# AgoraIO-Community/Solo

Hardware: AMD Instinct MI355X
Metric: 40 ms frames/sec (encode+decode) per GPU; concurrent real-time WB streams @1/2/4/8 MI355X (higher is better)
Workload: dtype int32 fixed point (int16 PCM, Q-format arithmetic, bit-exact); 1 GPU; BASELINE configs[2]: 4096 synthetic 16 kHz WB streams, full encode -> two-description bitstream -...; streams_per_gpu=4096, input_workers=16, launch=single process

## Files before the change

solo_amd/csrc/solo_api.hip:

```cpp
#include <hip/hip_runtime.h>
#include <vector>
#include <stdio.h>
#include <stdlib.h>
#include <string.h>
#include <new>

#include "../../include/solo_mi355x.h"
#include "solo_dec.h"

#define SOLO_CHECK(expr)                                        \
    do {                                                        \
        hipError_t e_ = (expr);                                 \
        if (e_ != hipSuccess) return -(int32_t)e_;              \
    } while (0)

#include "solo_dec_kernels.h"
#include "solo_l0_probe.h"
#include "solo_send.h"
#include "solo_mix.h"
#include "solo_mix_shared.h"
#include "solo_mix_selected.h"
#include "solo_fanout.h"
#include "solo_recv_report.h"
#include "solo_migrate.h"
// ... 102 lines not shown
        for (int t = 0; t < trips; t++) {
            if (t) x = sx_add(sx_add(x, a), sx_add(f, sx_add(g, (i32)(u32)h)));
            SOLO_WAVEOPS_CHAIN(x)
        }
        ROW(9, a); ROW(10, b); ROW(11, c); ROW(12, d); ROW(13, e); ROW(14, f); ROW(15, g); ROW(16, (u32)h); ROW(17, (u32)((u64)h >> 32));
    }
#undef ROW
#endif
}

__global__ void __launch_bounds__(256) solo_stream_list_check_kernel(const i32* map, int n, int n_streams, u32* verdict, i32* status) {
    __shared__ int bad;
    if (threadIdx.x == 0) bad = 0;
    __syncthreads();
    int mine = 0;
    for (int i = threadIdx.x; i < n; i += 256) {
        const i32 v = map[i];
        if (v < 0 || v >= n_streams || (i > 0 && map[i - 1] >= v)) mine = 1;
    }
    if (mine) atomicOr(&bad, 1);
    __syncthreads();
    const int verdict_bad = bad;
    if (threadIdx.x == 0) *verdict = (u32)verdict_bad;
    if (verdict_bad && status)
        for (int i = threadIdx.x; i < n; i += 256) status[i] = -1;
}

extern "C" const solo_dec_ops* solo_nb_dec_ops() { return &solo_dec_ops_table; }
extern "C" const solo_dec_ops* solo_wb_dec_ops();

#ifdef SOLO_WITH_ENCODER
#include "solo_enc_ops.h"
extern "C" int solo_launch_gate(const unsigned int* flag, unsigned int target, void* hip_stream);
extern "C" const solo_enc_ops* solo_nb_enc_ops();
extern "C" const solo_enc_ops* solo_wb_enc_ops();
#endif

#define SOLO_MAX_CHUNKS 64
enum {
    SOLO_VERDICT_ENC = 0,
    SOLO_VERDICT_DEC = 2,
    SOLO_VERDICT_RING,
    SOLO_VERDICT_SEND,
    SOLO_VERDICT_MIX,
    SOLO_VERDICT_REPORT,
    SOLO_VERDICT_EXPORT,
    SOLO_VERDICT_IMPORT,
    SOLO_N_VERDICTS = SOLO_VERDICT_IMPORT + 2
};
struct solo_batch {
    int32_t n_streams;
    int32_t slot;
    int have_enc, have_dec;
    USER_Ctrl_enc enc_ctrl;
    USER_Ctrl_dec dec_ctrl;
    void* d_enc_state;
#ifdef SOLO_WITH_ENCODER
    const solo_enc_ops* eops;
#endif
    void* d_nsq_ring;
    hipEvent_t evDecDone;
    int dec_done_recorded;
    void* d_parsed;
    size_t parsed_bytes;
    int dec_pipe_ready, dec_split, dec_chunk, dec_first;
    size_t dec_scratch_cap;
    void* d_rc_scratch;
    size_t rc_scratch_bytes;
    void* d_enc_work;
    int32_t enc_work_packets;
    int timing;
    hipEvent_t evDec[2];
    int ev_ready, ev_enc, ev_dec;
    int pipe_ready, chunk_packets;
    hipStream_t sA, sB, sC;
    hipEvent_t evFork, evJoinA[2], evJoinC[2], evA[SOLO_MAX_CHUNKS], evB[SOLO_MAX_CHUNKS], evC[SOLO_MAX_CHUNKS];
    int async_join;
    unsigned int enc_seq;
    unsigned long long join_cap[2];
    int evC_valid;
    int last_np, last_cp;
    hipEvent_t tev[3][SOLO_MAX_CHUNKS][2];
    int tev_ready, last_chunks;
    unsigned int* d_started;
    unsigned int started_target[SOLO_MAX_CHUNKS];
    int group_streams;
    int gate;
    int persist;
    int persist_group;
    unsigned int* d_flags;
    unsigned int ticket;
    unsigned int final_wait_ticks;
    int front_defer;
    void* d_nsq_stage;
    void* d_front_scratch;
    const solo_dec_ops* dops;
    void* d_dec_state;
    uint8_t* d_recv_ring;
    uint32_t* d_recv_lens;
    int32_t* d_recv_play;
    uint32_t* d_recv_stats;
    int32_t recv_depth, recv_slot;
    uint32_t* d_recv_trk;
    int recv_track;
    int32_t* d_recv_sel;
    uint32_t* d_verdict;
    void* d_send_scratch;
// ... 990 lines not shown
        const int32_t r = solo_wait_in_flight(b, st);
        if (r) return r;
    }
    uint32_t* verdict = b->d_verdict + SOLO_VERDICT_IMPORT;
    SOLO_CHECK(launch_list_check(d_streams, n, b->n_streams, verdict, NULL, st));
    SOLO_CHECK(solo_migrate_import_launch(migrate_handle(b), d_streams, n, which, d_blob, (long long)blob_stride, (SxMigCount*)d_count, verdict, st));
    return 0;
}

#ifdef SOLO_WITH_ENCODER
static int32_t solo_enc_pipe_setup(solo_batch* b) {
    const solo_enc_ops* ops = b->eops;
    int lo = 0, hi = 0;
    (void)hipDeviceGetStreamPriorityRange(&lo, &hi);
    SOLO_CHECK(hipStreamCreateWithPriority(&b->sA, hipStreamNonBlocking, lo));
    SOLO_CHECK(hipStreamCreateWithPriority(&b->sB, hipStreamNonBlocking, hi));
    SOLO_CHECK(hipStreamCreateWithPriority(&b->sC, hipStreamNonBlocking, lo));
    SOLO_CHECK(hipEventCreateWithFlags(&b->evFork, hipEventDisableTiming));
    for (int i = 0; i < 2; i++) {
        SOLO_CHECK(hipEventCreateWithFlags(&b->evJoinA[i], hipEventDisableTiming));
        SOLO_CHECK(hipEventCreateWithFlags(&b->evJoinC[i], hipEventDisableTiming));
    }
    for (int c = 0; c < SOLO_MAX_CHUNKS; c++) {
        SOLO_CHECK(hipEventCreateWithFlags(&b->evA[c], hipEventDisableTiming));
        SOLO_CHECK(hipEventCreateWithFlags(&b->evB[c], hipEventDisableTiming));
        SOLO_CHECK(hipEventCreateWithFlags(&b->evC[c], hipEventDisableTiming));
    }
    int dev = 0, ncu = 0;
    SOLO_CHECK(hipGetDevice(&dev));
    SOLO_CHECK(hipDeviceGetAttribute(&ncu, hipDeviceAttributeMultiprocessorCount, dev));
    b->persist = env_int("SOLO_ENC_PERSIST", 0) != 0;
    b->chunk_packets = env_int("SOLO_ENC_CHUNK", 1);
    if (b->chunk_packets < 0) b->chunk_packets = 1;
    b->gate = getenv("SOLO_ENC_GATE") ? (env_int("SOLO_ENC_GATE", 0) != 0) : -1;
    const int g_env = env_int("SOLO_ENC_GROUP", -1);
    b->group_streams = g_env >= 0 ? g_env : 8192;
    b->persist_group = g_env > 0 ? ((g_env + 3) & ~3) : ((ops->front_per_cu * (ncu > 0 ? ncu : 256)) & ~3);
    if (b->persist_group < 4) b->persist_group = 4;
    {
        const long us = env_int("SOLO_ENC_FINAL_WAIT_US", 20000);
        b->front_defer = us < 0;
        b->final_wait_ticks = (unsigned int)((us < 0 ? 0 : (us > 10000000 ? 10000000 : us)) * 100);
    }
    {
        int gs = (b->group_streams > 0 && b->group_streams < b->n_streams) ? b->group_streams : b->n_streams;
        if (b->persist && b->persist_group > gs) gs = b->persist_group < b->n_streams ? b->persist_group : b->n_streams;
        SOLO_CHECK(hipMalloc(&b->d_nsq_ring, ops->nsq_ring_bytes(gs)));
    }
    SOLO_CHECK(hipMalloc((void**)&b->d_started, SOLO_MAX_CHUNKS * sizeof(unsigned int)));
    SOLO_CHECK(hipMemset(b->d_started, 0, SOLO_MAX_CHUNKS * sizeof(unsigned int)));
    memset(b->started_target, 0, sizeof(b->started_target));
    if (b->persist) {
        const size_t nflags = (size_t)b->n_streams * 2 + (size_t)b->n_streams / 4 + 1 + 4;
        SOLO_CHECK(hipMalloc((void**)&b->d_flags, nflags * sizeof(unsigned int)));
        SOLO_CHECK(hipMemset(b->d_flags, 0, nflags * sizeof(unsigned int)));
        const int gs = b->persist_group < b->n_streams ? b->persist_group : b->n_streams;
        SOLO_CHECK(hipMalloc(&b->d_front_scratch, ops->front_scratch_bytes(gs)));
        SOLO_CHECK(hipMalloc(&b->d_nsq_stage, ops->nsq_stage_bytes(gs)));
    }
    b->ticket = 0;
    b->pipe_ready = 1;
    return 0;
}

static int32_t solo_encode_persist(solo_batch* b, const int16_t* d_pcm, int32_t n_packets, uint8_t* d_bits, int16_t* d_nbytes, int32_t* d_status,
                                   hipStream_t st, void* nin, void* nout, void* cin) {
// ... 66 lines not shown
    SOLO_CHECK(lerr);
    SOLO_CHECK(hipGetLastError());
    return 0;
}

static int32_t solo_encode_impl(solo_batch_t* b, const int32_t* map, int32_t n, const int16_t* d_pcm, int32_t n_packets, uint8_t* d_bits, int16_t* d_nbytes,
                                int32_t* d_status, hipStream_t st) {
    const size_t np = (size_t)b->n_streams * (size_t)n_packets;
    const solo_enc_ops* ops = b->eops;
    if (map && (unsigned long long)b->n_streams * (unsigned long long)ops->state_bytes >= (1ull << 32)) return -1;
    const unsigned long long per_wave = 64ull / (unsigned long long)ops->nsq_workgroups(64);
    if (((per_wave - 1ull) * 2ull * (unsigned long long)n_packets + 1ull) * (unsigned long long)ops->nsq_out_bytes >= (1ull << 32)) return -1;
    const size_t sz_in = np * 2 * ops->nsq_in_bytes, sz_out = np * 2 * ops->nsq_out_bytes, sz_code = np * ops->code_in_bytes;
    if (n_packets > b->enc_work_packets) {
        SOLO_CHECK(hipStreamSynchronize(st));
        if (b->pipe_ready) { (void)hipStreamSynchronize(b->sA); (void)hipStreamSynchronize(b->sB); (void)hipStreamSynchronize(b->sC); }
        dev_free(b->d_enc_work);
        SOLO_CHECK(hipMalloc(&b->d_enc_work, sz_in + sz_out + sz_code + 256));
        b->enc_work_packets = n_packets;
    }
    void* nin = b->d_enc_work;
    void* nout = (char*)b->d_enc_work + ((sz_in + 63) & ~(size_t)63);
    void* cin = (char*)nout + ((sz_out + 63) & ~(size_t)63);
    void* states = b->d_enc_state;
    if (!b->pipe_ready) {
        const int32_t r = solo_enc_pipe_setup(b);
        if (r) return r;
    }
    if (!map && b->persist && n_packets >= 2) return solo_encode_persist(b, d_pcm, n_packets, d_bits, d_nbytes, d_status, st, nin, nout, cin);

    int cp = b->chunk_packets > 0 ? b->chunk_packets : n_packets;
    int nchunks = (n_packets + cp - 1) / cp;
    if (nchunks > SOLO_MAX_CHUNKS) { cp = (n_packets + SOLO_MAX_CHUNKS - 1) / SOLO_MAX_CHUNKS; nchunks = (n_packets + cp - 1) / cp; }
    {
        const int gs = (b->group_streams > 0 && b->group_streams < b->n_streams) ? b->group_streams : b->n_streams;
        SOLO_CHECK(grow_scratch(b->d_rc_scratch, b->rc_scratch_bytes, ops->rc_scratch_bytes(gs, cp), b->sC));
    }
    const bool tm_req = b->timing && b->tev_ready;
    const unsigned long long cap = stream_capture(st);
    if (b->enc_seq > 0 && b->join_cap[(b->enc_seq - 1u) & 1u] != cap) b->evC_valid = -1;
    uint32_t* verdict = NULL;
    if (map) {
        if (b->evC_valid > 0) b->evC_valid = 0;
        verdict = b->d_verdict + SOLO_VERDICT_ENC + (b->enc_seq & 1u);
        if (b->enc_seq >= 2 && b->join_cap[b->enc_seq & 1u] == cap) {
            SOLO_CHECK(hipStreamWaitEvent(st, b->evJoinA[b->enc_seq & 1u], 0));
            SOLO_CHECK(hipStreamWaitEvent(st, b->evJoinC[b->enc_seq & 1u], 0));
        }
        SOLO_CHECK(launch_list_check(map, n, b->n_streams, verdict, d_status, st));
    }
    if (b->evC_valid < 0) b->evC_valid = 0;
    else if (b->enc_seq > 0 && (b->last_np != n_packets || b->last_cp != cp || b->evC_valid == 0)) {
        SOLO_CHECK(hipStreamWaitEvent(b->sA, b->evJoinC[(b->enc_seq - 1u) & 1u], 0));
        SOLO_CHECK(hipStreamWaitEvent(b->sB, b->evJoinA[(b->enc_seq - 1u) & 1u], 0));
        b->evC_valid = 0;
    }
    b->last_np = n_packets;
    b->last_cp = cp;
    SOLO_CHECK(hipEventRecord(b->evFork, st));
    SOLO_CHECK(hipStreamWaitEvent(b->sA, b->evFork, 0));
    SOLO_CHECK(hipStreamWaitEvent(b->sB, b->evFork, 0));
    SOLO_CHECK(hipStreamWaitEvent(b->sC, b->evFork, 0));
    const int nall = map ? n : b->n_streams;
    const int G = b->group_streams > 0 ? b->group_streams : nall;
    const int ngroups = (nall + G - 1) / G;
    const bool tm = tm_req && (size_t)ngroups * (size_t)nchunks <= SOLO_MAX_CHUNKS;
    const size_t frame_samples = (size_t)enc_packet_samples(b);
    int idx = 0;
    hipError_t lerr = hipSuccess;
    for (int g = 0; g < ngroups && lerr == hipSuccess; g++) {
        const int s0 = g * G, ns = (s0 + G <= nall) ? G : nall - s0;
        const size_t pk0 = (size_t)s0 * (size_t)n_packets;
        void* g_states = map ? states : (char*)states + (size_t)s0 * ops->state_bytes;
        const int32_t* g_map = map ? map + s0 : NULL;
        const int16_t* g_pcm = d_pcm + pk0 * frame_samples;
        void* g_nin = (char*)nin + pk0 * 2 * ops->nsq_in_bytes;
        void* g_nout = (char*)nout + pk0 * 2 * ops->nsq_out_bytes;
        void* g_cin = (char*)cin + pk0 * ops->code_in_bytes;
        uint8_t* g_bits = d_bits + pk0 * (size_t)b->slot;
        int16_t* g_nbytes = d_nbytes + pk0 * 2;
        int32_t* g_status = d_status ? d_status + s0 : NULL;
        for (int cc = 0; cc < nchunks; cc++, idx++) {
            const int c = idx % SOLO_MAX_CHUNKS, cprev = (idx + SOLO_MAX_CHUNKS - 1) % SOLO_MAX_CHUNKS;
            const int p0 = cc * cp, pc = (p0 + cp <= n_packets) ? cp : n_packets - p0;
            if (ngroups == 1 && cc < b->evC_valid) SOLO_CHECK(hipStreamWaitEvent(b->sA, b->evC[c], 0));
            if (idx > 0 && b->gate > 0) (void)solo_launch_gate(&b->d_started[cprev], b->started_target[cprev], b->sA);
            if (tm) (void)hipEventRecord(b->tev[0][c][0], b->sA);
            if ((lerr = ops->analysis(g_states, g_pcm, ns, n_packets, p0, pc, g_nin, g_cin, g_map, verdict, b->sA)) != hipSuccess) break;
            if (tm) (void)hipEventRecord(b->tev[0][c][1], b->sA);
            SOLO_CHECK(hipEventRecord(b->evA[c], b->sA));
            SOLO_CHECK(hipStreamWaitEvent(b->sB, b->evA[c], 0));
            if (tm) (void)hipEventRecord(b->tev[1][c][0], b->sB);
#ifdef SX_EXPERIMENTS
            static const int exp_skip = env_int("SOLO_EXP_SKIP", 0);
#else
            constexpr int exp_skip = 0;
#endif
            if (!(exp_skip & 1)) {
            if ((lerr = (hipError_t)ops->nsq(g_states, g_nin, g_nout, ns, n_packets, p0, pc, &b->d_started[c], b->d_nsq_ring, g_map, verdict, b->sB)) != hipSuccess) break;
            b->started_target[c] += (unsigned int)ops->nsq_workgroups(ns);
            }
            if (tm) (void)hipEventRecord(b->tev[1][c][1], b->sB);
            SOLO_CHECK(hipEventRecord(b->evB[c], b->sB));
            SOLO_CHECK(hipStreamWaitEvent(b->sC, b->evB[c], 0));
            if (tm) (void)hipEventRecord(b->tev[2][c][0], b->sC);
            if (!(exp_skip & 2))
            if ((lerr = ops->coding(g_states, g_cin, g_nout, ns, n_packets, p0, pc, b->slot, g_bits, g_nbytes, g_status, b->d_rc_scratch, g_map, verdict, b->sC)) != hipSuccess) break;
            if (tm) (void)hipEventRecord(b->tev[2][c][1], b->sC);
            SOLO_CHECK(hipEventRecord(b->evC[c], b->sC));
        }
    }
    const bool ok = lerr == hipSuccess;
    b->evC_valid = (ok && ngroups == 1 && !map) ? nchunks : 0;
    const int js = (int)(b->enc_seq & 1u);
    b->enc_seq++;
    b->join_cap[js] = cap;
    (void)hipEventRecord(b->evJoinA[js], b->sA);
    (void)hipEventRecord(b->evJoinC[js], b->sC);
    if (!b->async_join || !ok) {
        (void)hipStreamWaitEvent(st, b->evJoinA[js], 0);
        (void)hipStreamWaitEvent(st, b->evJoinC[js], 0);
    }
    if (!ok) {
        (void)hipEventRecord(b->evFork, b->sB);
        (void)hipStreamWaitEvent(st, b->evFork, 0);
    }
    b->last_chunks = !ok ? 0 : (tm ? ngroups * nchunks : (ngroups == 1 ? nchunks : 0));
    if (tm && ok) b->ev_enc = 1;
    SOLO_CHECK(lerr);
    SOLO_CHECK(hipGetLastError());
    return 0;
}
int32_t solo_batch_encode(solo_batch_t* b, const int16_t* d_pcm, int32_t n_packets, uint8_t* d_bits, int16_t* d_nbytes,
                          int32_t* d_status, void* hip_stream) {
    if (!b || !b->have_enc || !d_pcm || !d_bits || !d_nbytes || n_packets <= 0) return -1;
    return solo_encode_impl(b, NULL, 0, d_pcm, n_packets, d_bits, d_nbytes, d_status, (hipStream_t)hip_stream);
}
int32_t solo_batch_encode_streams(solo_batch_t* b, const int32_t* d_streams, int32_t n, const int16_t* d_pcm, int32_t n_packets, uint8_t* d_bits,
                                  int16_t* d_nbytes, int32_t* d_status, void* hip_stream) {
    if (!b || !b->have_enc || !d_streams || n <= 0 || n > b->n_streams || !d_pcm || !d_bits || !d_nbytes || n_packets <= 0) return -1;
    return solo_encode_impl(b, d_streams, n, d_pcm, n_packets, d_bits, d_nbytes, d_status, (hipStream_t)hip_stream);
}
#else
// ... 347 lines not shown
```

solo_amd/csrc/solo_enc_kernels.h:

```cpp
#pragma once
#include <hip/hip_runtime.h>
#include "solo_enc.h"
#include "solo_stream_ctl.h"

#ifndef SX_TU_FRONT
__global__ void __launch_bounds__(64) SX_K(solo_enc_init_kernel)(SxEncStream* states, int n_streams, int silk_rate_bps, int useMDIndex, int hb_joint, int useDTX, int fpp) {
    const int s = blockIdx.x;
    if (s >= n_streams) return;
    sx_enc_state_init(&states[s], silk_rate_bps, useMDIndex, hb_joint, useDTX, fpp);
}
__global__ void __launch_bounds__(64) SX_K(solo_enc_init_list_kernel)(SxEncStream* states, const SxStreamCtlList list, int n, int hb_joint, int fpp) {
    if ((int)blockIdx.x >= n) return;
    const SxStreamCtl r = list.r[blockIdx.x];
    sx_enc_state_init(&states[r.stream], r.a, r.b, hb_joint, r.c, fpp);
}
__global__ void __launch_bounds__(64) SX_K(solo_enc_ctl_list_kernel)(SxEncStream* states, const SxStreamCtlList list, int n) {
    if ((int)blockIdx.x >= n || SX_LANE != 0) return;
    const SxStreamCtl r = list.r[blockIdx.x];
    SxEncState* st = &states[r.stream].core;
    sx_enc_setup_rate(st, r.a);
    st->useMDIndex = r.b;
    st->useDTX = r.c;
}

// ... 97 lines not shown
    return total;
}

#ifndef SX_TU_FRONT
__global__ void __launch_bounds__(64) SX_K(solo_enc_rc_kernel)(const SxEncStream* states, const SxCodeIn* __restrict__ code_in,
                                                               const SxNsqOut* __restrict__ nsq_out, int n_streams, int n_packets, int p0, int pc,
                                                               u8* __restrict__ rcbuf, SxRcInfo* __restrict__ rcinfo, const u8* __restrict__ hbout,
                                                               int slot_bytes, u8* __restrict__ bits, i16* __restrict__ nbytes, i32* status,
                                                               const i32* __restrict__ map, const u32* verdict) {
    __shared__ SxRcWork w;
    if (sx_map_refused(map, verdict)) return;
    SX_K(sx_cdf_stage)(&w.cdf);
    const int lane = threadIdx.x, md = lane & 1;
    const int s = blockIdx.x * (SX_RC_LANES / 2) + (lane >> 1);
    if (lane >= SX_RC_LANES || s >= n_streams) return;
    const SxEncState* st = &states[map ? map[s] : s].core;
    const int useDTX = st->useDTX, useMDIndex = st->useMDIndex, fpp = st->fpp;
    const int hb_bytes = st->hb_joint ? 4 : 4 * fpp;
    i32 first_err = 0;
    for (int p = p0; p < p0 + pc; p++) {
        const size_t pk = (size_t)s * n_packets + p;
        const size_t slot = ((size_t)s * pc + (size_t)(p - p0)) * 2 + (size_t)md;
        const i32 ret = SX_K(sx_rc_code_and_assemble)(code_in[pk].idx, nsq_out + pk * 2, md, useDTX, useMDIndex, fpp, hb_bytes, &w.cdf, (u8*)&w.pw[lane][0],
                                                      rcbuf + slot * SX_RC_BUF_STRIDE, hbout + (slot & ~(size_t)1) * 4, slot_bytes, bits + pk * (size_t)slot_bytes,
                                                      nbytes + pk * 2, &rcinfo[slot]);
        if (ret < 0 && first_err == 0) first_err = ret;
    }
    if (status && md == 0) {
        if (p0 == 0) status[s] = first_err;
        else if (first_err != 0 && status[s] == 0) status[s] = first_err;
    }
}

__global__ void __launch_bounds__(64, SX_ANALYSIS_WAVES) SX_K(solo_enc_coding_kernel)(SxEncStream* states, const SxCodeIn* __restrict__ code_in,
                                                                const SxNsqOut* __restrict__ nsq_out, int n_streams, int n_packets, int p0,
                                                                int pc, u8* __restrict__ hbout, const i32* __restrict__ map, const u32* verdict) {
    __shared__ SxEncWork w;
    const int s = blockIdx.x;
    if (s >= n_streams || sx_map_refused(map, verdict)) return;
    SxEncStream* rec = &states[sx_map_stream(map, s)];
#if defined(SX_STOPS) && defined(__HIP_DEVICE_COMPILE__)
    SX_STOPS_ENTER(1)
#endif
    SX_K(solo_enc_enter)(&w, rec);
    for (int p = p0; p < p0 + pc; p++) {
        const size_t pk = (size_t)s * n_packets + p;
        const size_t rs = ((size_t)s * pc + (size_t)(p - p0)) * 2;
        sx_enc_stage_c_hb(rec, &w, code_in + pk, nsq_out + pk * 2);
        wv_sync();
        if (SX_LANE < 8) hbout[rs * 4 + SX_LANE] = w.hb_bytes[SX_LANE];
        wv_sync();
    }
}

#endif
#define SX_FRONT_RB SX_HB_Q
#ifndef SX_FRONT_PRIO
#define SX_FRONT_PRIO SX_ANALYSIS_PRIO
#endif
#ifndef SX_FRONT_POLL_SLEEPS
#define SX_FRONT_POLL_SLEEPS 4
#endif
struct SxFrontRcWork {
    SxCdf cdf;
    u32 pw[2 * SX_FRONT_RB][SX_RC_PW_ROW / 4];
};
// ... 133 lines not shown
    return sx_launch_ctl_batches(recs, n, [&](const SxStreamCtlList& l, int k) { hipLaunchKernelGGL(SX_K(solo_enc_init_list_kernel), dim3(k), dim3(64), 0, s, (SxEncStream*)states, l, k, hb_joint, fpp); });
}
static hipError_t SX_K(solo_enc_launch_ctl_list)(void* states, const SxStreamCtl* recs, int n, hipStream_t s) {
    return sx_launch_ctl_batches(recs, n, [&](const SxStreamCtlList& l, int k) { hipLaunchKernelGGL(SX_K(solo_enc_ctl_list_kernel), dim3(k), dim3(64), 0, s, (SxEncStream*)states, l, k); });
}
static hipError_t SX_K(solo_enc_launch_analysis)(void* states, const int16_t* pcm, int n_streams, int n_packets, int p0, int pc, void* nsq_in,
                                                 void* code_in, const int32_t* map, const uint32_t* verdict, hipStream_t s) {
    hipLaunchKernelGGL(SX_K(solo_enc_analysis_kernel), dim3(n_streams), dim3(64), 0, s, (SxEncStream*)states, pcm, n_streams, n_packets, p0, pc,
                       (SxNsqIn*)nsq_in, (SxCodeIn*)code_in, map, verdict);
    return hipGetLastError();
}
static size_t SX_K(solo_enc_rc_scratch_bytes)(int n_streams, int pc) {
    return (size_t)n_streams * (size_t)pc * 2 * (SX_RC_BUF_STRIDE + sizeof(SxRcInfo) + 4) + 128;
}
static SxRcInfo* SX_K(solo_enc_rcinfo_of)(u8* rcbuf, int n_streams, int pc) {
    return (SxRcInfo*)(rcbuf + (((size_t)n_streams * (size_t)pc * 2 * SX_RC_BUF_STRIDE + 63) & ~(size_t)63));
}
static u8* SX_K(solo_enc_hbout_of)(u8* rcbuf, int n_streams, int pc) {
    return (u8*)(SX_K(solo_enc_rcinfo_of)(rcbuf, n_streams, pc) + (size_t)n_streams * (size_t)pc * 2);
}
static hipError_t SX_K(solo_enc_launch_coding)(void* states, const void* code_in, const void* nsq_out, int n_streams, int n_packets, int p0, int pc,
                                               int slot, uint8_t* bits, int16_t* nbytes, int32_t* status, void* rc_scratch, const int32_t* map,
                                               const uint32_t* verdict, hipStream_t s) {
    u8* rcbuf = (u8*)rc_scratch;
    hipLaunchKernelGGL(SX_K(solo_enc_coding_kernel), dim3(n_streams), dim3(64), 0, s, (SxEncStream*)states, (const SxCodeIn*)code_in,
                       (const SxNsqOut*)nsq_out, n_streams, n_packets, p0, pc, SX_K(solo_enc_hbout_of)(rcbuf, n_streams, pc), map, verdict);
    hipError_t e = hipGetLastError();
    if (e != hipSuccess) return e;
    hipLaunchKernelGGL(SX_K(solo_enc_rc_kernel), dim3((n_streams + SX_RC_LANES / 2 - 1) / (SX_RC_LANES / 2)), dim3(64), 0, s, (const SxEncStream*)states, (const SxCodeIn*)code_in,
                       (const SxNsqOut*)nsq_out, n_streams, n_packets, p0, pc, rcbuf, SX_K(solo_enc_rcinfo_of)(rcbuf, n_streams, pc),
                       (const u8*)SX_K(solo_enc_hbout_of)(rcbuf, n_streams, pc), slot, bits, nbytes, status, map, verdict);
    return hipGetLastError();
}
#endif
#ifdef SX_TU_FRONT
extern "C" size_t SX_K(solo_enc_front_scratch_bytes)(int n_streams) { return (size_t)n_streams * (2 * SX_FRONT_RB) * SX_RC_BUF_STRIDE + 128; }
extern "C" hipError_t SX_K(solo_enc_launch_front)(void* states, const int16_t* pcm, int n_streams, int n_packets, void* nsq_in, void* code_in, const void* nsq_out,
                                              unsigned int* ana_flag, const unsigned int* nsq_flag, unsigned int* prog, unsigned int ticket0, int mode,
                                              unsigned int final_wait_ticks, int slot, uint8_t* bits, int16_t* nbytes, int32_t* status, void* scratch,
                                              unsigned int* started, hipStream_t s) {
    static bool lds_set = false;
    if (!lds_set) {
        const hipError_t e = hipFuncSetAttribute((const void*)SX_K(solo_enc_front_kernel), hipFuncAttributeMaxDynamicSharedMemorySize, (int)(SX_FRONT_WAVES * SX_FRONT_WORK_BYTES));
        if (e != hipSuccess) return e;
        lds_set = true;
    }
    hipLaunchKernelGGL(SX_K(solo_enc_front_kernel), dim3((n_streams + SX_FRONT_WAVES - 1) / SX_FRONT_WAVES), dim3(64 * SX_FRONT_WAVES), SX_FRONT_WAVES * SX_FRONT_WORK_BYTES, s, (SxEncStream*)states, pcm, n_streams, n_packets, (SxNsqIn*)nsq_in,
                       (SxCodeIn*)code_in, (const SxNsqOut*)nsq_out, ana_flag, nsq_flag, prog, ticket0, mode, final_wait_ticks, slot, bits, nbytes, status,
                       (u8*)scratch, started);
    return hipGetLastError();
}
#else
extern "C" size_t SX_K(solo_enc_front_scratch_bytes)(int n_streams);
extern "C" hipError_t SX_K(solo_enc_launch_front)(void* states, const int16_t* pcm, int n_streams, int n_packets, void* nsq_in, void* code_in, const void* nsq_out,
                                                  unsigned int* ana_flag, const unsigned int* nsq_flag, unsigned int* prog, unsigned int ticket0, int mode,
                                                  unsigned int final_wait_ticks, int slot, uint8_t* bits, int16_t* nbytes, int32_t* status, void* scratch,
                                                  unsigned int* started, hipStream_t s);
static const solo_enc_ops SX_K(solo_enc_ops_table) = {
    sizeof(SxEncStream), sizeof(SxNsqIn), sizeof(SxNsqOut), sizeof(SxCodeIn), SX_PACKET,
    SX_K(solo_enc_launch_init), SX_K(solo_enc_launch_init_list), SX_K(solo_enc_launch_ctl_list), SX_K(solo_enc_launch_analysis), SX_K(solo_launch_nsq), SX_K(solo_enc_launch_coding), SX_K(solo_enc_rc_scratch_bytes),
    SX_K(solo_nsq_workgroups), SX_K(solo_nsq_ring_bytes), SX_K(solo_enc_launch_front), SX_K(solo_launch_nsq_persist), SX_K(solo_enc_front_scratch_bytes), SX_K(solo_nsq_persist_workgroups), SX_K(solo_nsq_stage_bytes),
    SX_FRONT_WAVES, SX_FRONT_PER_CU};

#endif
```

solo_amd/csrc/solo_enc_ops.h:

```cpp
#pragma once
#include <hip/hip_runtime.h>
#include <stdint.h>
#include <stddef.h>
#include "solo_stream_ctl.h"
#ifndef SOLO_ENC_OPS_DEFINED
#define SOLO_ENC_OPS_DEFINED
struct solo_enc_ops {
    size_t state_bytes, nsq_in_bytes, nsq_out_bytes, code_in_bytes;
    int packet_samples;
    hipError_t (*init)(void* states, int n_streams, int silk_rate_bps, int useMDIndex, int hb_joint, int useDTX, int frames_per_packet, hipStream_t s);
    hipError_t (*init_list)(void* states, const SxStreamCtl* recs, int n, int hb_joint, int frames_per_packet, hipStream_t s);
    hipError_t (*ctl_list)(void* states, const SxStreamCtl* recs, int n, hipStream_t s);
    hipError_t (*analysis)(void* states, const int16_t* pcm, int n_streams, int n_packets, int p0, int pc, void* nsq_in, void* code_in, const int32_t* map,
                           const uint32_t* verdict, hipStream_t s);
    int (*nsq)(void* states, const void* in, void* out, int n_streams, int n_packets, int p0, int pc, unsigned int* started, void* ring, const int32_t* map,
               const uint32_t* verdict, void* hip_stream);
    hipError_t (*coding)(void* states, const void* code_in, const void* nsq_out, int n_streams, int n_packets, int p0, int pc, int slot,
                         uint8_t* bits, int16_t* nbytes, int32_t* status, void* rc_scratch, const int32_t* map, const uint32_t* verdict, hipStream_t s);
    size_t (*rc_scratch_bytes)(int n_streams, int pc);
    int (*nsq_workgroups)(int n_streams);
    size_t (*nsq_ring_bytes)(int n_streams);
    hipError_t (*front)(void* states, const int16_t* pcm, int n_streams, int n_packets, void* nsq_in, void* code_in, const void* nsq_out,
                        unsigned int* ana_flag, const unsigned int* nsq_flag, unsigned int* prog, unsigned int ticket0, int mode,
                        unsigned int final_wait_ticks, int slot, uint8_t* bits, int16_t* nbytes, int32_t* status, void* scratch,
                        unsigned int* started, hipStream_t s);
    int (*nsq_persist)(void* states, const void* in, void* out, int n_streams, int n_packets, unsigned int* started, void* ring,
                       const unsigned int* ana_flag, unsigned int* nsq_flag, unsigned int ticket0, unsigned int* err, void* stage, void* hip_stream);
    size_t (*front_scratch_bytes)(int n_streams);
    int (*nsq_persist_workgroups)(int n_streams);
    size_t (*nsq_stage_bytes)(int n_streams);
    int front_waves;
    int front_per_cu;
};
#endif
```

solo_amd/csrc/solo_nsq_row.hip:

```cpp
#define SX_GROUP 16
#define SX_PER_WAVE (64 / SX_GROUP)
#ifndef SX_NSQ_PERSIST_WAVES
#define SX_NSQ_PERSIST_WAVES 4
#endif
#if SX_NSQ_PERSIST_WAVES > 1
#define SX_SYNC_WAVE_ONLY 1
#endif
#include <hip/hip_runtime.h>
#include "solo_enc_nsq_row.h"

#ifndef SX_NSQ_PRIO
#define SX_NSQ_PRIO 3
#endif
#ifndef SX_NSQ_VGPR_CAP
#if SX_FS_KHZ == 16
#define SX_NSQ_VGPR_CAP 80
#else
#define SX_NSQ_VGPR_CAP 64
#endif
#endif
#if SX_NSQ_VGPR_CAP > 0
#define SX_NSQ_CAP_ATTR __attribute__((amdgpu_num_vgpr(SX_NSQ_VGPR_CAP)))
#else
#define SX_NSQ_CAP_ATTR
// ... 91 lines not shown
            const u32* src = (const u32*)&in[((size_t)wave * SX_PER_WAVE * n_packets + p) * 2 + f + (size_t)g * rec_stride];
            u32* dst = (u32*)&mine[f];
            constexpr int NW = (int)(sizeof(SxNsqIn) / 4), NU = (NW + SX_GROUP - 1) / SX_GROUP;
            u32 v[NU];
#pragma unroll
            for (int u = 0; u < NU; u++) { const int i = u * SX_GROUP + SX_LANE; v[u] = i < NW ? sx_pub_ld(&src[i]) : 0u; }
#pragma unroll
            for (int u = 0; u < NU; u++) { const int i = u * SX_GROUP + SX_LANE; if (i < NW) dst[i] = v[u]; }
        }
        wv_sync();
        for (int f = 0; f < fpp; f++) {
            const size_t r0 = ((size_t)wave * SX_PER_WAVE * n_packets + p) * 2 + f;
            sx_nsq_del_dec(Pu, pOff, &mine[f], (char*)&out[r0], (u32)g * rec_stride * (u32)sizeof(SxNsqOut), wg, rgu, (u32)(g * SX_GROUP), 64);
            wv_sync();
        }
        static_assert(sizeof(SxNsqOut) % 4 == 0, "dword copy of the output records");
        for (int f = 0; f < fpp; f++) {
            u32* rec = (u32*)&out[((size_t)wave * SX_PER_WAVE * n_packets + p) * 2 + f + (size_t)g * rec_stride];
            u32 v[(sizeof(SxNsqOut) / 4 + SX_GROUP - 1) / SX_GROUP];
#pragma unroll
            for (int u = 0; u < (int)(sizeof(v) / 4); u++) { const int i = u * SX_GROUP + SX_LANE; v[u] = i < (int)(sizeof(SxNsqOut) / 4) ? rec[i] : 0u; }
#pragma unroll
            for (int u = 0; u < (int)(sizeof(v) / 4); u++) { const int i = u * SX_GROUP + SX_LANE; if (i < (int)(sizeof(SxNsqOut) / 4)) sx_pub_st(&rec[i], v[u]); }
        }
        sx_pub_drain();
        if (lane == 0) sx_flag_st(&nsq_flag[wave], target);
        if (p == 0) SX_NSQ_TRACE(1, wall_clock64())
    }
    SX_NSQ_TRACE(2, wall_clock64())
    SX_NSQ_TRACE(3, waited_)
}

#if SX_FS_KHZ == 8
extern "C" __global__ void __launch_bounds__(64) solo_gate_kernel(const unsigned int* flag, unsigned int target) {
    if (threadIdx.x == 0) {
        for (int it = 0; it < 20000; it++) {
            if (__atomic_load_n(flag, __ATOMIC_RELAXED) - target < 0x80000000u) break;
            __builtin_amdgcn_s_sleep(32);
        }
    }
}
extern "C" int solo_launch_gate(const unsigned int* flag, unsigned int target, void* hip_stream) {
    hipLaunchKernelGGL(solo_gate_kernel, dim3(1), dim3(64), 0, (hipStream_t)hip_stream, flag, target);
    return (int)hipGetLastError();
}

extern "C" __global__ void __launch_bounds__(64) solo_debug_rowops_kernel(const i32* in, const i32* idx, i32* out) {
#if defined(__HIP_DEVICE_COMPILE__)
    const int lane = threadIdx.x;
    i32 v[1] = {in[lane]}, ix[1] = {idx[lane] & 3}, d[1] = {-1}, mv[1], mi[1];
    RWT_FROM(d, v, 0) out[0 * 64 + lane] = d[0];
    RWT_FROM(d, v, 1) out[1 * 64 + lane] = d[0];
    RWT_FROM(d, v, 2) out[2 * 64 + lane] = d[0];
    d[0] = -1; RWT_TO0(d, v, 1) out[3 * 64 + lane] = d[0];
    d[0] = -1; RWT_TO0(d, v, 2) out[4 * 64 + lane] = d[0];
    RWT_SUM(d, v) out[5 * 64 + lane] = d[0];
    RWT_OR(d, v) out[6 * 64 + lane] = d[0];
    RWK_GATHER(d, v, ix) out[7 * 64 + lane] = d[0];
    RWK_ARGMIN(v, mv, mi) out[8 * 64 + lane] = mv[0]; out[9 * 64 + lane] = mi[0];
    RWK_ARGMAX(v, mv, mi) out[10 * 64 + lane] = mv[0]; out[11 * 64 + lane] = mi[0];
    RWS_SUM(v, d) out[12 * 64 + lane] = d[0];
    out[13 * 64 + lane] = rwk_from(v[0], ix[0]);
#endif
}
extern "C" __global__ void __launch_bounds__(64) solo_debug_clock_kernel(unsigned long long* out2, int iters, int* sink) {
    int a = threadIdx.x, b = blockIdx.x | 1;
    const unsigned long long c0 = __builtin_readcyclecounter(), w0 = wall_clock64();
    for (int r = 0; r < iters; r++) {
#pragma unroll
        for (int u = 0; u < 64; u++) a = a * b + u;
    }
    const unsigned long long c1 = __builtin_readcyclecounter(), w1 = wall_clock64();
    if (a == 0x7F123457) *sink = a;
    if (blockIdx.x == 0 && threadIdx.x == 0) { out2[0] = c1 - c0; out2[1] = w1 - w0; }
}
extern "C" int32_t solo_debug_clock(double* mhz_out) {
    int dev = 0, ncu = 0;
    if (hipGetDevice(&dev) != hipSuccess || hipDeviceGetAttribute(&ncu, hipDeviceAttributeMultiprocessorCount, dev) != hipSuccess) return -1;
// ... 45 lines not shown
```

Before: 4.274 million 40ms packets/s (encode+decode).

## Batch range-coding across chunks and defer HB stage behind next NSQ

Splits the encoder's per-chunk coding into a header/HB kernel and a batched range-coding kernel. The batched kernel codes up to SOLO_ENC_RC_BATCH packets per stream in one launch, packing several streams per wave. The third-stage work is also deferred by one chunk and gated on the next NSQ having started, so it overlaps with NSQ. The aim is fewer small launches and better lane use, at the cost of larger scratch, extra gate kernels and more complex error and status handling.

Result: faster. 4.433 million 40ms packets/s (encode+decode), median of 6 (+3.7%).

```diff
diff --git a/solo_amd/csrc/solo_api.hip b/solo_amd/csrc/solo_api.hip
--- a/solo_amd/csrc/solo_api.hip
+++ b/solo_amd/csrc/solo_api.hip
@@ -158,11 +158,14 @@
 #ifdef SOLO_WITH_ENCODER
 #include "solo_enc_ops.h"
 extern "C" int solo_launch_gate(const unsigned int* flag, unsigned int target, void* hip_stream);
+extern "C" int solo_launch_gate_for(const unsigned int* flag, unsigned int target, int max_iters, void* hip_stream);
 extern "C" const solo_enc_ops* solo_nb_enc_ops();
 extern "C" const solo_enc_ops* solo_wb_enc_ops();
 #endif
 
 #define SOLO_MAX_CHUNKS 64
+#define SOLO_ENC_RC_BATCH_DEFAULT 5
+#define SOLO_HB_GATE_ITERS 500
 enum {
     SOLO_VERDICT_ENC = 0,
     SOLO_VERDICT_DEC = 2,
@@ -199,6 +202,7 @@
     hipEvent_t evDec[2];
     int ev_ready, ev_enc, ev_dec;
     int pipe_ready, chunk_packets;
+    int rc_batch;
     hipStream_t sA, sB, sC;
     hipEvent_t evFork, evJoinA[2], evJoinC[2], evA[SOLO_MAX_CHUNKS], evB[SOLO_MAX_CHUNKS], evC[SOLO_MAX_CHUNKS];
     int async_join;
@@ -1255,6 +1259,9 @@
     b->persist = env_int("SOLO_ENC_PERSIST", 0) != 0;
     b->chunk_packets = env_int("SOLO_ENC_CHUNK", 1);
     if (b->chunk_packets < 0) b->chunk_packets = 1;
+    b->rc_batch = env_int("SOLO_ENC_RC_BATCH", SOLO_ENC_RC_BATCH_DEFAULT);
+    if (b->rc_batch < 1) b->rc_batch = 1;
+    if (b->rc_batch > ops->rc_batch_max) b->rc_batch = ops->rc_batch_max;
     b->gate = getenv("SOLO_ENC_GATE") ? (env_int("SOLO_ENC_GATE", 0) != 0) : -1;
     const int g_env = env_int("SOLO_ENC_GROUP", -1);
     b->group_streams = g_env >= 0 ? g_env : 8192;
@@ -1387,12 +1394,14 @@
     int cp = b->chunk_packets > 0 ? b->chunk_packets : n_packets;
     int nchunks = (n_packets + cp - 1) / cp;
     if (nchunks > SOLO_MAX_CHUNKS) { cp = (n_packets + SOLO_MAX_CHUNKS - 1) / SOLO_MAX_CHUNKS; nchunks = (n_packets + cp - 1) / cp; }
+    const unsigned long long cap = stream_capture(st);
+    const int kc = nchunks > 1 && !cap && b->rc_batch / cp > 1 ? (b->rc_batch / cp < nchunks ? b->rc_batch / cp : nchunks) : 1;
+    const int kb_cap = kc * cp;
     {
         const int gs = (b->group_streams > 0 && b->group_streams < b->n_streams) ? b->group_streams : b->n_streams;
-        SOLO_CHECK(grow_scratch(b->d_rc_scratch, b->rc_scratch_bytes, ops->rc_scratch_bytes(gs, cp), b->sC));
+        SOLO_CHECK(grow_scratch(b->d_rc_scratch, b->rc_scratch_bytes, ops->rc_scratch_bytes(gs, kb_cap), b->sC));
     }
     const bool tm_req = b->timing && b->tev_ready;
-    const unsigned long long cap = stream_capture(st);
     if (b->enc_seq > 0 && b->join_cap[(b->enc_seq - 1u) & 1u] != cap) b->evC_valid = -1;
     uint32_t* verdict = NULL;
     if (map) {
@@ -1423,6 +1432,11 @@
     const size_t frame_samples = (size_t)enc_packet_samples(b);
     int idx = 0;
     hipError_t lerr = hipSuccess;
+#ifdef SX_EXPERIMENTS
+    static const int exp_skip = env_int("SOLO_EXP_SKIP", 0);
+#else
+    constexpr int exp_skip = 0;
+#endif
     for (int g = 0; g < ngroups && lerr == hipSuccess; g++) {
         const int s0 = g * G, ns = (s0 + G <= nall) ? G : nall - s0;
         const size_t pk0 = (size_t)s0 * (size_t)n_packets;
@@ -1435,6 +1449,25 @@
         uint8_t* g_bits = d_bits + pk0 * (size_t)b->slot;
         int16_t* g_nbytes = d_nbytes + pk0 * 2;
         int32_t* g_status = d_status ? d_status + s0 : NULL;
+        int pb = 0, hb_end = 0, idx_b = idx;
+        int pend = -1, pend_idx = 0;
+        auto third = [&](int tcc, int tidx) -> hipError_t {
+            const int tc = tidx % SOLO_MAX_CHUNKS, tp0 = tcc * cp, tpc = (tp0 + cp <= n_packets) ? cp : n_packets - tp0;
+            const bool last = (tcc + 1) % kc == 0 || tcc + 1 == nchunks;
+            hipError_t e;
+            if (tm) (void)hipEventRecord(b->tev[2][tc][0], b->sC);
+            if (!(exp_skip & 2) && (e = ops->hb(g_states, g_cin, g_nout, ns, n_packets, tp0, tpc, pb, kb_cap, cp, b->d_rc_scratch, g_map, verdict, b->sC)) != hipSuccess) return e;
+            hb_end = tp0 + tpc;
+            if (last && !(exp_skip & 6) &&
+                (e = ops->rc_batch(g_states, g_cin, g_nout, ns, n_packets, pb, hb_end - pb, kb_cap, cp, b->slot, g_bits, g_nbytes, g_status, b->d_rc_scratch, g_map, verdict, b->sC)) != hipSuccess) return e;
+            if (tm) (void)hipEventRecord(b->tev[2][tc][1], b->sC);
+            if (last) {
+                for (int i = idx_b; i <= tidx; i++) if ((e = hipEventRecord(b->evC[i % SOLO_MAX_CHUNKS], b->sC)) != hipSuccess) return e;
+                pb = hb_end;
+                idx_b = tidx + 1;
+            }
+            return hipSuccess;
+        };
         for (int cc = 0; cc < nchunks; cc++, idx++) {
             const int c = idx % SOLO_MAX_CHUNKS, cprev = (idx + SOLO_MAX_CHUNKS - 1) % SOLO_MAX_CHUNKS;
             const int p0 = cc * cp, pc = (p0 + cp <= n_packets) ? cp : n_packets - p0;
@@ -1446,17 +1479,26 @@
             SOLO_CHECK(hipEventRecord(b->evA[c], b->sA));
             SOLO_CHECK(hipStreamWaitEvent(b->sB, b->evA[c], 0));
             if (tm) (void)hipEventRecord(b->tev[1][c][0], b->sB);
-#ifdef SX_EXPERIMENTS
-            static const int exp_skip = env_int("SOLO_EXP_SKIP", 0);
-#else
-            constexpr int exp_skip = 0;
-#endif
             if (!(exp_skip & 1)) {
             if ((lerr = (hipError_t)ops->nsq(g_states, g_nin, g_nout, ns, n_packets, p0, pc, &b->d_started[c], b->d_nsq_ring, g_map, verdict, b->sB)) != hipSuccess) break;
             b->started_target[c] += (unsigned int)ops->nsq_workgroups(ns);
             }
             if (tm) (void)hipEventRecord(b->tev[1][c][1], b->sB);
             SOLO_CHECK(hipEventRecord(b->evB[c], b->sB));
+            if (kc > 1 || (exp_skip & 4)) {
+                if (kc <= 1 || (exp_skip & 1)) {
+                    SOLO_CHECK(hipStreamWaitEvent(b->sC, b->evB[c], 0));
+                    if ((lerr = third(cc, idx)) != hipSuccess) break;
+                } else {
+                    if (pend >= 0) {
+                        SOLO_CHECK(hipStreamWaitEvent(b->sC, b->evB[cprev], 0));
+                        (void)solo_launch_gate_for(&b->d_started[c], b->started_target[c], SOLO_HB_GATE_ITERS, b->sC);
+                        if ((lerr = third(pend, pend_idx)) != hipSuccess) break;
+                    }
+                    pend = cc; pend_idx = idx;
+                }
+                continue;
+            }
             SOLO_CHECK(hipStreamWaitEvent(b->sC, b->evB[c], 0));
             if (tm) (void)hipEventRecord(b->tev[2][c][0], b->sC);
             if (!(exp_skip & 2))
@@ -1464,6 +1506,13 @@
             if (tm) (void)hipEventRecord(b->tev[2][c][1], b->sC);
             SOLO_CHECK(hipEventRecord(b->evC[c], b->sC));
         }
+        if (pend >= 0) {
+            (void)hipStreamWaitEvent(b->sC, b->evB[pend_idx % SOLO_MAX_CHUNKS], 0);
+            const hipError_t e = third(pend, pend_idx);
+            if (lerr == hipSuccess) lerr = e;
+        }
+        if (lerr != hipSuccess && kc > 1 && hb_end > pb)
+            (void)ops->rc_batch(g_states, g_cin, g_nout, ns, n_packets, pb, hb_end - pb, kb_cap, cp, b->slot, g_bits, g_nbytes, g_status, b->d_rc_scratch, g_map, verdict, b->sC);
     }
     const bool ok = lerr == hipSuccess;
     b->evC_valid = (ok && ngroups == 1 && !map) ? nchunks : 0;
diff --git a/solo_amd/csrc/solo_enc_kernels.h b/solo_amd/csrc/solo_enc_kernels.h
--- a/solo_amd/csrc/solo_enc_kernels.h
+++ b/solo_amd/csrc/solo_enc_kernels.h
@@ -153,6 +153,39 @@
     }
 }
 
+__global__ void __launch_bounds__(64) SX_K(solo_enc_rc_batch_kernel)(const SxEncStream* states, const SxCodeIn* __restrict__ code_in,
+                                                                     const SxNsqOut* __restrict__ nsq_out, int n_streams, int n_packets, int pb, int kb,
+                                                                     int kb_cap, int cp, u8* __restrict__ rcbuf, SxRcInfo* __restrict__ rcinfo,
+                                                                     const u8* __restrict__ hbout, int slot_bytes, u8* __restrict__ bits,
+                                                                     i16* __restrict__ nbytes, i32* status, const i32* __restrict__ map, const u32* verdict) {
+    __shared__ SxRcWork w;
+    if (sx_map_refused(map, verdict)) return;
+    SX_K(sx_cdf_stage)(&w.cdf);
+    const int lane = threadIdx.x, per = 2 * kb, spw = 64 / per;
+    const int sl = lane / per, r = lane - sl * per, j = r >> 1, md = r & 1;
+    const int s = blockIdx.x * spw + sl;
+    const bool on = sl < spw && s < n_streams;
+    i32 ret = 0;
+    if (on) {
+        const SxEncState* st = &states[map ? map[s] : s].core;
+        const int useDTX = st->useDTX, useMDIndex = st->useMDIndex, fpp = st->fpp;
+        const int hb_bytes = st->hb_joint ? 4 : 4 * fpp;
+        const int ci = j / cp, pin = j - ci * cp, left = n_packets - (pb + ci * cp), pcc = left < cp ? left : cp;
+        const size_t pk = (size_t)s * n_packets + (size_t)(pb + j);
+        const size_t slot = ((size_t)s * kb_cap + (size_t)j) * 2 + (size_t)md;
+        ret = SX_K(sx_rc_code_and_assemble)(code_in[pk].idx, nsq_out + pk * 2, md, useDTX, useMDIndex, fpp, hb_bytes, &w.cdf, (u8*)&w.pw[lane][0],
+                                            rcbuf + slot * SX_RC_BUF_STRIDE, hbout + ((size_t)ci * n_streams * cp + (size_t)s * pcc + (size_t)pin) * 8, slot_bytes,
+                                            bits + pk * (size_t)slot_bytes, nbytes + pk * 2, &rcinfo[slot]);
+    }
+    const unsigned long long bad = __builtin_amdgcn_ballot_w64(on && ret < 0) >> (sl < spw ? sl * per : 0);
+    const unsigned long long mine = per < 64 ? (bad & ((1ull << per) - 1ull)) : bad;
+    const i32 first_err = __shfl(ret, sl * per + (mine ? (int)__builtin_ctzll(mine) : 0));
+    if (status && on && r == 0) {
+        if (pb == 0) status[s] = mine ? first_err : 0;
+        else if (mine && status[s] == 0) status[s] = first_err;
+    }
+}
+
 __global__ void __launch_bounds__(64, SX_ANALYSIS_WAVES) SX_K(solo_enc_coding_kernel)(SxEncStream* states, const SxCodeIn* __restrict__ code_in,
                                                                 const SxNsqOut* __restrict__ nsq_out, int n_streams, int n_packets, int p0,
                                                                 int pc, u8* __restrict__ hbout, const i32* __restrict__ map, const u32* verdict) {
@@ -352,6 +385,24 @@
                        (const u8*)SX_K(solo_enc_hbout_of)(rcbuf, n_streams, pc), slot, bits, nbytes, status, map, verdict);
     return hipGetLastError();
 }
+static hipError_t SX_K(solo_enc_launch_hb)(void* states, const void* code_in, const void* nsq_out, int n_streams, int n_packets, int p0, int pc, int pb, int kb_cap,
+                                           int cp, void* rc_scratch, const int32_t* map, const uint32_t* verdict, hipStream_t s) {
+    u8* hbout = SX_K(solo_enc_hbout_of)((u8*)rc_scratch, n_streams, kb_cap) + (size_t)((p0 - pb) / cp) * (size_t)n_streams * (size_t)cp * 8;
+    hipLaunchKernelGGL(SX_K(solo_enc_coding_kernel), dim3(n_streams), dim3(64), 0, s, (SxEncStream*)states, (const SxCodeIn*)code_in,
+                       (const SxNsqOut*)nsq_out, n_streams, n_packets, p0, pc, hbout, map, verdict);
+    return hipGetLastError();
+}
+static hipError_t SX_K(solo_enc_launch_rc_batch)(void* states, const void* code_in, const void* nsq_out, int n_streams, int n_packets, int pb, int kb, int kb_cap,
+                                                 int cp, int slot, uint8_t* bits, int16_t* nbytes, int32_t* status, void* rc_scratch, const int32_t* map,
+                                                 const uint32_t* verdict, hipStream_t s) {
+    if (kb < 1 || kb > SX_RC_LANES / 2 || kb > kb_cap || cp < 1) return hipErrorInvalidValue;
+    u8* rcbuf = (u8*)rc_scratch;
+    const int spw = SX_RC_LANES / (2 * kb);
+    hipLaunchKernelGGL(SX_K(solo_enc_rc_batch_kernel), dim3((n_streams + spw - 1) / spw), dim3(64), 0, s, (const SxEncStream*)states, (const SxCodeIn*)code_in,
+                       (const SxNsqOut*)nsq_out, n_streams, n_packets, pb, kb, kb_cap, cp, rcbuf, SX_K(solo_enc_rcinfo_of)(rcbuf, n_streams, kb_cap),
+                       (const u8*)SX_K(solo_enc_hbout_of)(rcbuf, n_streams, kb_cap), slot, bits, nbytes, status, map, verdict);
+    return hipGetLastError();
+}
 #endif
 #ifdef SX_TU_FRONT
 extern "C" size_t SX_K(solo_enc_front_scratch_bytes)(int n_streams) { return (size_t)n_streams * (2 * SX_FRONT_RB) * SX_RC_BUF_STRIDE + 128; }
@@ -380,6 +431,6 @@
     sizeof(SxEncStream), sizeof(SxNsqIn), sizeof(SxNsqOut), sizeof(SxCodeIn), SX_PACKET,
     SX_K(solo_enc_launch_init), SX_K(solo_enc_launch_init_list), SX_K(solo_enc_launch_ctl_list), SX_K(solo_enc_launch_analysis), SX_K(solo_launch_nsq), SX_K(solo_enc_launch_coding), SX_K(solo_enc_rc_scratch_bytes),
     SX_K(solo_nsq_workgroups), SX_K(solo_nsq_ring_bytes), SX_K(solo_enc_launch_front), SX_K(solo_launch_nsq_persist), SX_K(solo_enc_front_scratch_bytes), SX_K(solo_nsq_persist_workgroups), SX_K(solo_nsq_stage_bytes),
-    SX_FRONT_WAVES, SX_FRONT_PER_CU};
-
-#endif
+    SX_FRONT_WAVES, SX_FRONT_PER_CU, SX_K(solo_enc_launch_hb), SX_K(solo_enc_launch_rc_batch), SX_RC_LANES / 2};
+
+#endif
diff --git a/solo_amd/csrc/solo_enc_ops.h b/solo_amd/csrc/solo_enc_ops.h
--- a/solo_amd/csrc/solo_enc_ops.h
+++ b/solo_amd/csrc/solo_enc_ops.h
@@ -31,5 +31,10 @@
     size_t (*nsq_stage_bytes)(int n_streams);
     int front_waves;
     int front_per_cu;
+    hipError_t (*hb)(void* states, const void* code_in, const void* nsq_out, int n_streams, int n_packets, int p0, int pc, int pb, int kb_cap, int cp,
+                     void* rc_scratch, const int32_t* map, const uint32_t* verdict, hipStream_t s);
+    hipError_t (*rc_batch)(void* states, const void* code_in, const void* nsq_out, int n_streams, int n_packets, int pb, int kb, int kb_cap, int cp, int slot,
+                           uint8_t* bits, int16_t* nbytes, int32_t* status, void* rc_scratch, const int32_t* map, const uint32_t* verdict, hipStream_t s);
+    int rc_batch_max;
 };
 #endif
diff --git a/solo_amd/csrc/solo_nsq_row.hip b/solo_amd/csrc/solo_nsq_row.hip
--- a/solo_amd/csrc/solo_nsq_row.hip
+++ b/solo_amd/csrc/solo_nsq_row.hip
@@ -147,18 +147,19 @@
 }
 
 #if SX_FS_KHZ == 8
-extern "C" __global__ void __launch_bounds__(64) solo_gate_kernel(const unsigned int* flag, unsigned int target) {
+extern "C" __global__ void __launch_bounds__(64) solo_gate_kernel(const unsigned int* flag, unsigned int target, int max_iters) {
     if (threadIdx.x == 0) {
-        for (int it = 0; it < 20000; it++) {
+        for (int it = 0; it < max_iters; it++) {
             if (__atomic_load_n(flag, __ATOMIC_RELAXED) - target < 0x80000000u) break;
             __builtin_amdgcn_s_sleep(32);
         }
     }
 }
-extern "C" int solo_launch_gate(const unsigned int* flag, unsigned int target, void* hip_stream) {
-    hipLaunchKernelGGL(solo_gate_kernel, dim3(1), dim3(64), 0, (hipStream_t)hip_stream, flag, target);
-    return (int)hipGetLastError();
-}
+extern "C" int solo_launch_gate_for(const unsigned int* flag, unsigned int target, int max_iters, void* hip_stream) {
+    hipLaunchKernelGGL(solo_gate_kernel, dim3(1), dim3(64), 0, (hipStream_t)hip_stream, flag, target, max_iters);
+    return (int)hipGetLastError();
+}
+extern "C" int solo_launch_gate(const unsigned int* flag, unsigned int target, void* hip_stream) { return solo_launch_gate_for(flag, target, 20000, hip_stream); }
 
 extern "C" __global__ void __launch_bounds__(64) solo_debug_rowops_kernel(const i32* in, const i32* idx, i32* out) {
 #if defined(__HIP_DEVICE_COMPILE__)
```
